# mcbuehler/DeepSEE

Measured on AMD Instinct MI355X. Metric: train-step images/sec (G+D fwd+bwd), 8x 32->256 bs=8, higher is better.
Workload: dtype fp32

## Files before the change

deepsee_amd/csrc/coarse.cpp:

```cpp
#include <hip/hip_runtime.h>
#include <stdint.h>

#include <initializer_list>
#include <vector>

#include "../../include/deepsee_hip.h"

void dsee_set_error(const char* fmt, ...);

namespace {

constexpr int kHidden = 128;
constexpr long kAmaxFloats = 64 * 32;
constexpr double kWgradF16x2MinFlop = 1e9;

#define DSEE_TRY(call)          \
  do {                          \
    const int rc__ = (call);    \
    if (rc__ != DSEE_OK) return rc__; \
  } while (0)

inline size_t up256(size_t b) { return (b + 255) / 256 * 256; }

struct Arena {
// ... 45 lines not shown
                 int C, hipStream_t stream) {
  const int has_t = nl.table != nullptr, ld = kHidden + (has_t ? 32 : 0), rows = 2 * C;
  if (!b.tab_ready) DSEE_TRY(dsee_onehot_conv3x3_pack(nl.w_shared, b.tab, kHidden, label_nc, stream));
  DSEE_TRY(dsee_onehot_conv3x3_fwd(labels, b.tab, nl.b_shared, b.cat, N, lab_h, lab_w, shift, label_nc, kHidden, ld, 0, 1,
                                   has_t ? kHidden : -1, b.amax_cat, has_t ? 1.0f : 0.0f, stream));
  if (from == kStatsOfX)
    DSEE_TRY(dsee_norm_stats(x, N, H * W, C, 1, eps, momentum, b.mean, b.invstd, nl.running_mean, nl.running_var, b.stats, stream));
  else if (from == kStatsOfParts)
    DSEE_TRY(dsee_norm_stats_finalize_parts(part, dsee_stats_part_rows((long)N * (H / 4) * (W / 4) * (C / 4)), C, eps, momentum,
                                            b.mean, b.invstd, nl.running_mean, nl.running_var, stream));
  else
    DSEE_TRY(dsee_norm_eval_stats(nl.running_mean, nl.running_var, C, eps, b.mean, b.invstd, stream));
  if (b.wp_direct) {
    const dsee_conv_geom g = {N, H, W, ld, H, W, rows, 3, 3, 1, -1, 1, 0, 0, 1};
    return dsee_conv2d_modulate_fwd(&g, b.cat, b.wp_direct, nl.table, kHidden, nl.bias_packed, x, b.mean, b.invstd, b.out_h,
                                    b.out_scale, C, nl.add_one, slope, stream);
  }
  DSEE_TRY(dsee_wino43_input_f16x2(b.cat, b.v2, N, H, W, ld, b.amax_cat, DSEE_WINO_V_BOUND, stream));
  if (!b.u_ready && !b.u_bound_ready) {
    DSEE_TRY(dsee_absmax(nl.w2a, (long)rows * kHidden * 9, b.amax_u, stream));
    if (has_t) DSEE_TRY(dsee_absmax(nl.table, (long)N * 9 * rows * 32, b.amax_u, stream));
  }
  if (has_t)
    DSEE_TRY(dsee_wino43_weights_table(nl.w2a, nl.table, reinterpret_cast<float*>(b.u2), N, rows, kHidden, 2, b.amax_u, stream));
  else if (!b.u_ready)
    DSEE_TRY(dsee_wino43_weights(nl.w2a, reinterpret_cast<float*>(b.u2), rows, kHidden, 0, 2, b.amax_u, stream));
  return dsee_spade_fused_fwd(b.v2, b.u2, b.amax_cat, DSEE_WINO_V_BOUND, b.amax_u, nl.bias_packed, x, b.mean, b.invstd, b.out_h,
                              b.out_scale, N, H, W, C, rows, ld, has_t ? N : 1, nl.add_one, slope, b.amax_h, b.amax_xhat, b.sign_mask,
                              stream);
}

int gemm_nt(const void* a2, const void* b2, float* c, long M, int Nn, int K, long rpg, int brows, const float* amax_a, float bound,
            const float* amax_b, hipStream_t st) {
  if (Nn % 256 == 0 && K % 32 == 0) return dsee_gemm_f16x2_pre_w4(a2, b2, c, M, Nn, K, rpg, brows, amax_a, bound, amax_b, st);
  return dsee_gemm_f16x2_pre(a2, b2, c, M, Nn, K, rpg, brows, amax_a, bound, amax_b, st);
}

int wino_conv3x3_product(const float* h, const float* amax_h, const float* w, float* amax_w, uint16_t* v2, uint16_t* u2, float* m,
                         bool choose_gemm, int N, int H, int W, int C, hipStream_t stream) {
  const long T = (long)N * (H / 4) * (W / 4);
  DSEE_TRY(dsee_absmax(w, (long)C * C * 9, amax_w, stream));
  DSEE_TRY(dsee_wino43_weights(w, reinterpret_cast<float*>(u2), C, C, 0, 2, amax_w, stream));
  DSEE_TRY(dsee_wino43_input_f16x2(h, v2, N, H, W, C, amax_h, DSEE_WINO_V_BOUND, stream));
  return (choose_gemm ? gemm_nt : dsee_gemm_f16x2_pre)(v2, u2, m, 36 * T, C, C, T, C, amax_h, DSEE_WINO_V_BOUND, amax_w, stream);
}

struct InferScratch {
  size_t norm_bytes;
  float *h, *dx0, *stat, *amax_h, *amax_w, *m;
  uint16_t *v2, *u2;
};
// ... 902 lines not shown
```

deepsee_amd/csrc/spade_fused.hip:

```cpp
#include <stdlib.h>

#include <type_traits>
#include <utility>

#include "dsee_common.h"

#ifndef DSEE_FUSED_ABL
#define DSEE_FUSED_ABL 0
#endif

#ifndef DSEE_FUSED_SCHED
#define DSEE_FUSED_SCHED 0
#endif

#ifndef DSEE_FUSED_SET_A
#define DSEE_FUSED_SET_A 4
#endif
#define DSEE_FUSED_SET_B (32 / DSEE_FUSED_SET_A)

#ifndef DSEE_FUSED_W16_DEFAULT
#define DSEE_FUSED_W16_DEFAULT 0
#endif

namespace {
// ... 31 lines not shown
    tg = (sup / rh) * DSEE_FUSED_SET_A + (in / DSEE_FUSED_SET_B);
    rg = (int)(sup % rh) * DSEE_FUSED_SET_B + (in % DSEE_FUSED_SET_B);
  } else {
    tg = l / rgn;
    rg = (int)(l % rgn);
  }
  const long t0 = tg * 64;
  const int n = (int)(t0 / a.tpi);
  const int g = a.G > 1 ? n : 0;

  const float sv = dsee_pow2_scale(a.v_bound * dsee_amax_read(a.amax_v));
  const float su = dsee_pow2_scale(dsee_amax_read(a.amax_u));
  const float oscale = 1.f / (sv * su);

  const int dr = 8 * wave + (lane >> 3);
  const int dcc = (lane & 7) ^ ((dr >> 1) & 7);
  const int dslab = dcc >> 2;
  const unsigned dlo = (unsigned)(dr * 64 + (dcc & 3) * 16);
  const unsigned voffu = dlo + (unsigned)dslab * (unsigned)a.u_slab_bytes;
  const unsigned voffv = dlo + (unsigned)dslab * (unsigned)a.v_slab_bytes;
  const unsigned voffu_l = dslab ? 0xFFFFFFF0u : voffu, voffv_l = dslab ? 0xFFFFFFF0u : voffv;
  const __amdgpu_buffer_rsrc_t rsu = __builtin_amdgcn_make_buffer_rsrc((void*)uniform_ptr(a.U2), 0, (int)a.u_bytes, 0x00020000);
  const __amdgpu_buffer_rsrc_t rsv = __builtin_amdgcn_make_buffer_rsrc((void*)uniform_ptr(a.V2), 0, (int)a.v_bytes, 0x00020000);
  const unsigned PU = (unsigned)(a.G * a.u_group_bytes), PV = (unsigned)(a.T * 64);
  const unsigned QU = (unsigned)(2 * a.u_slab_bytes), QV = (unsigned)(2 * a.v_slab_bytes);
  const unsigned base_u = (unsigned)((long)g * a.u_group_bytes + (long)rg * 4096), base_v = (unsigned)(t0 * 64);
  auto dma_u = [&](int par, int pc, unsigned opos) {
    unsigned char* dst = smem + (par * NP + pc) * PIECE + wave * 1024;
    __builtin_amdgcn_raw_ptr_buffer_load_lds(rsu, (__attribute__((address_space(3))) void*)dst, 16,
                                             (HALF_LAST && pc == NP - 1) ? voffu_l : voffu, opos + pc * QU, 0, 0);
  };
  auto dma_v = [&](int par, int pc, unsigned opos) {
    unsigned char* dst = smem + UREG + (par * NP + pc) * PIECE + wave * 1024;
    __builtin_amdgcn_raw_ptr_buffer_load_lds(rsv, (__attribute__((address_space(3))) void*)dst, 16,
                                             (HALF_LAST && pc == NP - 1) ? voffv_l : voffv, opos + pc * QV, 0, 0);
  };

  const int fi = lane & 15, oc = lane >> 4;
  auto foff = [&](int r, int t) {
    const int chunk = PK ? 4 * t + oc : 4 * (oc >> 1) + 2 * t + (oc & 1);
    return (unsigned)((8 * r + (chunk ^ ((r >> 1) & 7))) * 16);
  };
  const int rga = 16 * wq + fi, rtv = 16 * wt + fi;
  const unsigned au0 = foff(rga, 0), au1 = foff(rga, 1), au0h = au0 + 7 * PIECE, au1h = au1 + 7 * PIECE;
  const unsigned av0 = UREG + foff(rtv, 0), av1 = UREG + foff(rtv, 1), av0h = av0 + 7 * PIECE, av1h = av1 + 7 * PIECE;
  struct Frag {
    u32x4 g0, g1, b0, b1, v0, v1;
  };
  auto ldf = [&](Frag& f, auto par_c, auto pc_c) {
    constexpr int so = (decltype(par_c)::value * NP + decltype(pc_c)::value) * PIECE;
    constexpr bool hi = so >= 7 * PIECE;
    constexpr int io = hi ? so - 7 * PIECE : so;
    static_assert(io >= 0 && io + 4096 + PIECE <= 65536, "window");
// ... 437 lines not shown
  } else {
    tg = l / rgn;
    rg = (int)(l % rgn);
  }
  const long t0 = tg * 64;
  const int n = (int)(t0 / a.tpi);
  const int g = a.G > 1 ? n : 0;

  const float sv = dsee_pow2_scale(a.v_bound * dsee_amax_read(a.amax_v));
  const float su = dsee_pow2_scale(dsee_amax_read(a.amax_u));
  const float oscale = 1.f / (sv * su);

  const bool dma_v = wave >= 8;
  const int dw = wave & 7;
  const int dr = 8 * dw + (lane >> 3);
  const int dcc = (lane & 7) ^ ((dr >> 1) & 7);
  const int dslab = dcc >> 2;
  const unsigned dlo = (unsigned)(dr * 64 + (dcc & 3) * 16);
  const unsigned slab_bytes = (unsigned)(dma_v ? a.v_slab_bytes : a.u_slab_bytes);
  const unsigned voff = dlo + (unsigned)dslab * slab_bytes;
  const unsigned voff_l = dslab ? 0xFFFFFFF0u : voff;
  const __amdgpu_buffer_rsrc_t rs = __builtin_amdgcn_make_buffer_rsrc(
      (void*)uniform_ptr(dma_v ? a.V2 : a.U2), 0, (int)(dma_v ? a.v_bytes : a.u_bytes), 0x00020000);
  const unsigned PP_ = dma_v ? (unsigned)(a.T * 64) : (unsigned)(a.G * a.u_group_bytes);
  const unsigned QQ_ = 2 * slab_bytes;
  const unsigned base_o = dma_v ? (unsigned)(t0 * 64) : (unsigned)((long)g * a.u_group_bytes + (long)rg * 4096);
  unsigned char* const dbase = smem + (dma_v ? UREG : 0) + dw * 1024;
  auto dma = [&](int par, int pc, unsigned opos) {
    unsigned char* dst = dbase + (par * NP + pc) * PIECE;
    __builtin_amdgcn_raw_ptr_buffer_load_lds(rs, (__attribute__((address_space(3))) void*)dst, 16,
                                             (HALF_LAST && pc == NP - 1) ? voff_l : voff, opos + pc * QQ_, 0, 0);
  };

  const int fi = lane & 15, oc = lane >> 4;
  auto foff = [&](int r, int t) {
    const int chunk = PK ? 4 * t + oc : 4 * (oc >> 1) + 2 * t + (oc & 1);
    return (unsigned)((8 * r + (chunk ^ ((r >> 1) & 7))) * 16);
  };
  const int rga = 16 * wb + fi, rtv = 16 * wt + fi;
  const unsigned au0 = foff(rga, 0), au1 = foff(rga, 1);
  const unsigned av0 = UREG + foff(rtv, 0), av1 = UREG + foff(rtv, 1);
  struct Frag {
    u32x4 a0, a1, v0, v1;
  };
  auto ldf = [&](Frag& f, auto par_c, auto pc_c) {
    constexpr int so = (decltype(par_c)::value * NP + decltype(pc_c)::value) * PIECE;
    constexpr bool hi = so >= 7 * PIECE;
    constexpr int io = hi ? so - 7 * PIECE : so;
    static_assert(io >= 0 && io + PIECE <= 65536, "window");
    const unsigned w0 = hi ? 7 * PIECE : 0;
    f.a0 = *reinterpret_cast<const u32x4*>(smem + (au0 + w0) + io);
    f.a1 = *reinterpret_cast<const u32x4*>(smem + (au1 + w0) + io);
    f.v0 = *reinterpret_cast<const u32x4*>(smem + (av0 + w0) + io);
    f.v1 = *reinterpret_cast<const u32x4*>(smem + (av1 + w0) + io);
// ... 237 lines not shown
    }
  }
  if (a.amax_xhat) {
#pragma unroll
    for (int o = 32; o > 0; o >>= 1) xmax = fmaxf(xmax, __shfl_xor(xmax, o, 64));
    if (lane == 0) {
      unsigned* line = reinterpret_cast<unsigned*>(a.amax_xhat + ((blockIdx.x * 16 + wave) & (DSEE_AMAX_LINES - 1)) * DSEE_AMAX_STRIDE);
      const unsigned bits = __builtin_bit_cast(unsigned, xmax);
      if (bits > __hip_atomic_load(line, __ATOMIC_RELAXED, __HIP_MEMORY_SCOPE_AGENT)) atomicMax(line, bits);
    }
  }
#endif
}

}

static float* g_fused_stamps = nullptr;

#if DSEE_FUSED_ABL
extern "C" void dsee_fused_set_stamps(float* p) { g_fused_stamps = p; }
#endif


static int spade_fused_launch(bool packed, const void* V2, const void* U2, const float* amax_cat, float v_bound,
                              const float* amax_u, const float* bias_packed, const float* x, const float* mean,
                              const float* invstd, float* out_h, float* out_scale, int N, int H, int W, int C, int rows, int K,
                              int groups, int stat_groups, float add_one, float slope, float* amax_h, float* amax_xhat,
                              unsigned* sign_mask, hipStream_t st) {
  DSEE_CHECK_ARG(V2 && U2 && amax_cat && amax_u && x && mean && invstd && out_h);
  DSEE_CHECK_ARG(rows == 2 * C && C % 32 == 0 && H % 4 == 0 && W % 4 == 0 && (K == 128 || K == 160));
  DSEE_CHECK_ARG(groups == 1 || groups == N);
  DSEE_CHECK_ARG(stat_groups == 1 || stat_groups == N);
  const int tpi = (H / 4) * (W / 4);
  DSEE_CHECK_ARG(tpi % 64 == 0);
  const long T = (long)N * tpi;
  FusedArgs a;
  a.V2 = (const unsigned char*)V2;
  a.U2 = (const unsigned char*)U2;
  a.amax_v = amax_cat;
  a.amax_u = amax_u;
  a.bias = bias_packed;
  a.x = x;
  a.mean = mean;
  a.invstd = invstd;
  a.stat_ld = stat_groups == 1 ? 0 : C;
  a.out = out_h;
  a.scale = out_scale;
  a.mask = sign_mask;
  a.cshift = 0;
  while ((4 << a.cshift) < 4 * C) ++a.cshift;
  a.cshift += 2;
  DSEE_CHECK_ARG(!sign_mask || (C & (C - 1)) == 0);
  DSEE_CHECK_ARG((long)N * H * W * C < (1L << 30));
  a.amax_h = amax_h;
  a.amax_xhat = amax_xhat;
  a.T = T;
  a.v_slab_bytes = 36L * T * 64;
  a.u_slab_bytes = (long)rows * 64;
  const int kslab = packed ? 32 : 16;
  a.u_group_bytes = (long)(K / kslab) * rows * 64;
  const long vb = a.v_slab_bytes * (K / kslab), ub = a.u_group_bytes * 36 * groups;
  DSEE_CHECK_ARG(vb < 0xFFFFFFF0L && ub < 0xFFFFFFF0L);
  a.v_bytes = (unsigned)vb;
  a.u_bytes = (unsigned)ub;
  a.tpi = tpi;
  a.tw = W / 4;
  a.H = H;
  a.W = W;
  a.C = C;
  a.rows = rows;
  a.G = groups;
  a.v_bound = v_bound;
  a.add_one = add_one;
  a.slope = slope;
  a.stamps = g_fused_stamps;
  const long ntile = (T / 64) * (rows / 64);
  DSEE_CHECK_ARG(ntile < 0x7FFFFFFF);
  const int np = packed ? (K + 63) / 64 : K / 32;
  const int rd = packed ? 3 : 2;
  const size_t lds = (size_t)rd * np * 16384;
  const char* const w16_env = getenv("DSEE_FUSED_W16");
  const int w16 = w16_env ? atoi(w16_env) : DSEE_FUSED_W16_DEFAULT;
#define DSEE_FUSED_K(KERNEL, THREADS, NP, WS, PKD)                                                                   \
  do {                                                                                                               \
    static bool attr_done = false;                                                                                   \
    if (!attr_done) {                                                                                                \
      hipError_t e = hipFuncSetAttribute(reinterpret_cast<const void*>(&KERNEL<NP, WS, PKD, (PKD ? 3 : 2)>),         \
                                         hipFuncAttributeMaxDynamicSharedMemorySize, (int)lds);                     \
      if (e != hipSuccess) {                                                                                         \
        dsee_set_error("hipFuncSetAttribute(%zu bytes of LDS): %s", lds, hipGetErrorString(e));                     \
        return DSEE_ELAUNCH;                                                                                         \
      }                                                                                                              \
      attr_done = true;                                                                                              \
    }                                                                                                                \
    KERNEL<NP, WS, PKD, (PKD ? 3 : 2)><<<(int)ntile, THREADS, lds, st>>>(a);                                         \
  } while (0)
#define DSEE_FUSED(NP, WS, PKD)                                                                                      \
  do {                                                                                                               \
    if (w16)                                                                                                         \
      DSEE_FUSED_K(spade_fused_fwd16_kernel, 1024, NP, WS, PKD);                                                     \
    else                                                                                                             \
// ... 2 lines not shown
  if (packed) {
    if (np == 3) {
      if (out_scale) DSEE_FUSED(3, true, true); else DSEE_FUSED(3, false, true);
    } else {
      if (out_scale) DSEE_FUSED(2, true, true); else DSEE_FUSED(2, false, true);
    }
  } else if (np == 5) {
    if (out_scale) DSEE_FUSED(5, true, false); else DSEE_FUSED(5, false, false);
  } else {
    if (out_scale) DSEE_FUSED(4, true, false); else DSEE_FUSED(4, false, false);
  }
#undef DSEE_FUSED
#undef DSEE_FUSED_K
  DSEE_LAUNCH_CHECK();
  return DSEE_OK;
}

extern "C" {

int dsee_spade_fused_fwd(const void* V2, const void* U2, const float* amax_cat, float v_bound, const float* amax_u,
                         const float* bias_packed, const float* x, const float* mean, const float* invstd, float* out_h,
                         float* out_scale, int N, int H, int W, int C, int rows, int K, int groups, float add_one,
                         float slope, float* amax_h, float* amax_xhat, uint32_t* sign_mask, hipStream_t st) {
  return spade_fused_launch(false, V2, U2, amax_cat, v_bound, amax_u, bias_packed, x, mean, invstd, out_h, out_scale, N, H, W,
                            C, rows, K, groups, 1, add_one, slope, amax_h, amax_xhat, sign_mask, st);
}

int dsee_spade_fused_fwd_f16p(const void* V1, const void* U1, const float* amax_cat, float v_bound, const float* amax_u,
                              const float* bias_packed, const float* x, const float* mean, const float* invstd, float* out_h,
                              float* out_scale, int N, int H, int W, int C, int rows, int K, int groups, float add_one,
                              float slope, float* amax_h, float* amax_xhat, uint32_t* sign_mask, hipStream_t st) {
  return spade_fused_launch(true, V1, U1, amax_cat, v_bound, amax_u, bias_packed, x, mean, invstd, out_h, out_scale, N, H, W,
                            C, rows, K, groups, 1, add_one, slope, amax_h, amax_xhat, sign_mask, st);
}

int dsee_spade_fused_fwd_sg(const void* V2, const void* U2, const float* amax_cat, float v_bound, const float* amax_u,
                            const float* bias_packed, const float* x, const float* mean, const float* invstd, float* out_h,
                            float* out_scale, int N, int H, int W, int C, int rows, int K, int groups, int stat_groups,
                            float add_one, float slope, float* amax_h, float* amax_xhat, uint32_t* sign_mask, hipStream_t st) {
  return spade_fused_launch(false, V2, U2, amax_cat, v_bound, amax_u, bias_packed, x, mean, invstd, out_h, out_scale, N, H, W,
                            C, rows, K, groups, stat_groups, add_one, slope, amax_h, amax_xhat, sign_mask, st);
}

int dsee_spade_fused_fwd_f16p_sg(const void* V1, const void* U1, const float* amax_cat, float v_bound, const float* amax_u,
                                 const float* bias_packed, const float* x, const float* mean, const float* invstd,
                                 float* out_h, float* out_scale, int N, int H, int W, int C, int rows, int K, int groups,
                                 int stat_groups, float add_one, float slope, float* amax_h, float* amax_xhat,
                                 uint32_t* sign_mask, hipStream_t st) {
  return spade_fused_launch(true, V1, U1, amax_cat, v_bound, amax_u, bias_packed, x, mean, invstd, out_h, out_scale, N, H, W,
                            C, rows, K, groups, stat_groups, add_one, slope, amax_h, amax_xhat, sign_mask, st);
}

}
```

deepsee_amd/csrc/spade_fused_args.h:

```cpp
#pragma once
#include <type_traits>
#include <utility>

#include "dsee_common.h"

namespace {

typedef _Float16 f16x8 __attribute__((ext_vector_type(8)));
typedef unsigned u32x4 __attribute__((ext_vector_type(4)));

struct FusedArgs {
  const unsigned char* V2;
  const unsigned char* U2;
  const float* amax_v;
  const float* amax_u;
  const float* bias;
  const float* x;
  const float* mean;
  const float* invstd;
  int stat_ld;
  float* out;
  float* amax_h;
  float* amax_xhat;
  float* scale;
  int cshift;
  unsigned* mask;
  long T;
  long v_slab_bytes, u_slab_bytes, u_group_bytes;
  unsigned v_bytes, u_bytes;
  int tpi, tw;
  int H, W, C, rows;
  int G;
  float v_bound, add_one, slope;
  float* stamps;
};

template <int I>
using ic = std::integral_constant<int, I>;
template <class F, int... Is>
__device__ __forceinline__ void static_for_impl(F&& f, std::integer_sequence<int, Is...>) {
  (f(ic<Is>{}), ...);
}
template <int N, class F>
__device__ __forceinline__ void static_for(F&& f) {
  static_for_impl(f, std::make_integer_sequence<int, N>{});
}

__device__ __forceinline__ const unsigned char* uniform_ptr(const unsigned char* p) {
  const unsigned long long v = (unsigned long long)p;
  const unsigned lo = __builtin_amdgcn_readfirstlane((unsigned)v), hi = __builtin_amdgcn_readfirstlane((unsigned)(v >> 32));
  return (const unsigned char*)(((unsigned long long)hi << 32) | lo);
// ... 5 lines not shown
```

deepsee_amd/csrc/winograd.hip:

```cpp
#include "dsee_common.h"
#include "dsee_rng.h"

namespace {

typedef unsigned short u16x4 __attribute__((ext_vector_type(4)));
__device__ __forceinline__ void split3(float x, unsigned short (&h)[3]) {
  const __bf16 b0 = (__bf16)x;
  const float r1 = x - (float)b0;
  const __bf16 b1 = (__bf16)r1;
  const __bf16 b2 = (__bf16)(r1 - (float)b1);
  h[0] = __builtin_bit_cast(unsigned short, b0);
  h[1] = __builtin_bit_cast(unsigned short, b1);
  h[2] = __builtin_bit_cast(unsigned short, b2);
}
__device__ __forceinline__ size_t split_index(size_t row, int k, size_t rows, int p) {
  return (((size_t)(k >> 4) * rows + row) * 3 + p) * 16 + (k & 15);
}
__device__ __forceinline__ void store_split4(unsigned short* base, size_t row, int k, size_t rows, const f32x4& v) {
  unsigned short h[4][3];
#pragma unroll
  for (int e = 0; e < 4; ++e) split3(v[e], h[e]);
#pragma unroll
  for (int p = 0; p < 3; ++p) {
    const u16x4 w = {h[0][p], h[1][p], h[2][p], h[3][p]};
// ... 1015 lines not shown
#pragma unroll
  for (int j = 0; j < 8; ++j) {
    const float x = v[j] * sc;
    h0[j] = (_Float16)x;
    h1[j] = (_Float16)(x - (float)h0[j]);
  }
  auto pk = [](_Float16 a, _Float16 b) {
    return (unsigned)__builtin_bit_cast(unsigned short, a) | ((unsigned)__builtin_bit_cast(unsigned short, b) << 16);
  };
  const dsee_u32x4 w0 = {pk(h0[0], h0[1]), pk(h0[2], h0[3]), pk(h0[4], h0[5]), pk(h0[6], h0[7])};
  _Float16* Uh = reinterpret_cast<_Float16*>(U);
  if (split == 2) {
    const dsee_u32x4 w1 = {pk(h1[0], h1[1]), pk(h1[2], h1[3]), pk(h1[4], h1[5]), pk(h1[6], h1[7])};
    _Float16* o = Uh + block * per * 2 + (((size_t)(k0 >> 4) * rows + row) * 2) * 16 + (k0 & 15);
    *reinterpret_cast<dsee_u32x4*>(o) = w0;
    *reinterpret_cast<dsee_u32x4*>(o + 16) = w1;
  } else if (split == 3) {
    *reinterpret_cast<dsee_u32x4*>(Uh + block * per + ((size_t)(k0 >> 4) * rows + row) * 16 + (k0 & 15)) = w0;
  } else {
    *reinterpret_cast<dsee_u32x4*>(Uh + block * per + ((size_t)(k0 >> 5) * rows + row) * 32 + (k0 & 31)) = w0;
  }
}

__global__ __launch_bounds__(256) void wino43_weight_table8_kernel(const float* __restrict__ w2a, const float* __restrict__ table,
                                                                   float* __restrict__ U, int N, int rows, int ca, int Kpad,
                                                                   int split, const float* __restrict__ amax) {
  const unsigned K8 = (unsigned)Kpad >> 3;
  const size_t per = (size_t)rows * Kpad;
  const long total = (long)N * rows * K8;
  const float sc = split >= 2 ? dsee_pow2_scale(dsee_amax_read(amax)) : 1.f;
  for (long i = blockIdx.x * (long)blockDim.x + threadIdx.x; i < total; i += (long)gridDim.x * blockDim.x) {
    const unsigned iu = (unsigned)i, rr = iu / K8, n = rr / (unsigned)rows;
    const int k0 = (int)(iu - rr * K8) * 8, row = (int)(rr - n * (unsigned)rows);
    float g[8][9];
    if (k0 < ca) {
      const f32x4* src = reinterpret_cast<const f32x4*>(w2a + ((size_t)row * ca + k0) * 9);
#pragma unroll
      for (int q = 0; q < 18; ++q) {
        const f32x4 v = src[q];
#pragma unroll
        for (int e = 0; e < 4; ++e) g[(q * 4 + e) / 9][(q * 4 + e) % 9] = v[e];
      }
    } else if (k0 < ca + 32) {
#pragma unroll
      for (int tap = 0; tap < 9; ++tap) {
        const float* src = table + (((size_t)n * 9 + tap) * rows + row) * 32 + (k0 - ca);
        const f32x4 a = *reinterpret_cast<const f32x4*>(src), b = *reinterpret_cast<const f32x4*>(src + 4);
#pragma unroll
        for (int e = 0; e < 4; ++e) {
          g[e][tap] = a[e];
          g[4 + e][tap] = b[e];
        }
      }
    } else {
#pragma unroll
      for (int j = 0; j < 8; ++j)
#pragma unroll
        for (int tap = 0; tap < 9; ++tap) g[j][tap] = 0.f;
    }
    ggt8(g, [&](int xi, const float (&v)[8]) { store_u8(U, split, (size_t)xi * N + n, per, rows, Kpad, row, k0, sc, v); });
  }
}

__global__ __launch_bounds__(256) void wino43_weight8_kernel(const float* __restrict__ w, float* __restrict__ U, int Cout, int Cin,
                                                             int rows, int Kpad, int transpose_flip, int split,
                                                             const float* __restrict__ amax, long w_stride, long u_stride) {
  w += (size_t)blockIdx.y * w_stride;
  U += (size_t)blockIdx.y * u_stride;
  if (amax) amax += (size_t)blockIdx.y * (DSEE_AMAX_LINES * DSEE_AMAX_STRIDE);
  const unsigned K8 = (unsigned)Kpad >> 3;
  const size_t per = (size_t)rows * Kpad;
  const long total = (long)rows * K8;
  const float sc = split >= 2 ? dsee_pow2_scale(dsee_amax_read(amax)) : 1.f;
  const int R = transpose_flip ? Cin : Cout, K = transpose_flip ? Cout : Cin;
  for (long i = blockIdx.x * (long)blockDim.x + threadIdx.x; i < total; i += (long)gridDim.x * blockDim.x) {
    const unsigned iu = (unsigned)i, row = iu / K8;
    const int k0 = (int)(iu - row * K8) * 8;
    float g[8][9];
#pragma unroll
    for (int j = 0; j < 8; ++j) {
      const int k = k0 + j;
      const bool ok = (int)row < R && k < K;
      const int co = transpose_flip ? k : (int)row, ci = transpose_flip ? (int)row : k;
// ... 401 lines not shown
                                   int stat_groups, float add_one, float slope, const float* mscale, hipStream_t st) {
  DSEE_CHECK_ARG(stat_groups == 1 || stat_groups == N);
  const int stat_ld = stat_groups == 1 ? 0 : C;
  DSEE_CHECK_ARG(wino_items32(N, H, W, C));
  DSEE_CHECK_ARG(M && x && mean && invstd && out_h && C % 64 == 0 && rows == 2 * C);
  DSEE_CHECK_ARG(H % 4 == 0 && W % 4 == 0);
  DSEE_CHECK_ARG((long)N * (H / 4) * (W / 4) * rows * 4 < 0xFFFFFFF0L);
  const int grid = wgrid((long)N * (H / 4) * (W / 4) * (C / 4));
  if (mscale)
    wino43_output_modulate_kernel<<<grid, 256, 0, st>>>(reinterpret_cast<const _Float16*>(M), bias_packed, x, mean, invstd,
                                                        out_h, out_scale, N, H, W, C, rows, add_one, slope, mscale, stat_ld);
  else
    wino43_output_modulate_kernel<<<grid, 256, 0, st>>>(M, bias_packed, x, mean, invstd, out_h, out_scale, N, H, W, C, rows,
                                                        add_one, slope, nullptr, stat_ld);
  DSEE_LAUNCH_CHECK();
  return DSEE_OK;
}

int dsee_wino43_weights_table(const float* w2a, const float* table, float* U, int N, int rows, int ca, int split,
                              const float* amax_w, hipStream_t st) {
  DSEE_CHECK_ARG(table && U && (ca == 0 || w2a) && ca % 32 == 0 && rows % 128 == 0 && (split < 2 || amax_w));
  const int Kpad = dsee_conv_kpad(1, 1, ca + 32);
  if (split != 1 && Kpad % 8 == 0)
    wino43_weight_table8_kernel<<<wgrid((long)N * rows * Kpad / 8), 256, 0, st>>>(w2a, table, U, N, rows, ca, Kpad, split,
                                                                                  amax_w);
  else
    wino43_weight_table_kernel<<<wgrid((long)N * rows * Kpad), 256, 0, st>>>(w2a, table, U, N, rows, ca, Kpad, split,
                                                                             amax_w);
  DSEE_LAUNCH_CHECK();
  return DSEE_OK;
}

}
```

deepsee_amd/ops.py:

```python
import os
import ctypes as C

import threading
from collections import namedtuple
from typing import NamedTuple, Optional

import torch

from . import lib as L
from .plan import KernelPlan, DEFAULT_PLAN, current as P

LRELU_SLOPE = 0.2
BN_EPS = 1e-5
BN_MOMENTUM = 0.1
SN_EPS = 1e-12
NHIDDEN = 128

_scratch = {}

PROFILE = None
PROFILE_BYTES = {}
PROFILE_OPERAND_GB = 0.0


# ... 1705 lines not shown
def _norm_cat(w_sh, b_sh, labels, shift, n, h, w, has_a, has_t, cat_ups):
    nc, ca = labels.nc, (NHIDDEN if has_a else 0)
    ld = ca + (32 if has_t else 0)
    cat, actv_low = new(n, h, w, ld), None
    cat_amax = amax_slot()
    if has_a:
        tab = new(9, nc, NHIDDEN)
        L.call("onehot_conv3x3_pack", w_sh.contiguous(), tab, NHIDDEN, nc)
        if cat_ups:
            assert not has_t and ld == NHIDDEN
            actv_low = new(n, h >> cat_ups, w >> cat_ups, NHIDDEN)
            L.call("onehot_conv3x3_fwd", labels.t, tab, b_sh, actv_low, n, labels.h, labels.w, shift, nc, NHIDDEN,
                   NHIDDEN, 0, 1, -1, cat_amax, 0.0)
            L.call("upsample_noise_fwd", actv_low, None, None, cat, n, h, w, NHIDDEN, cat_ups)
        else:
            L.call("onehot_conv3x3_fwd", labels.t, tab, b_sh, cat, n, labels.h, labels.w, shift, nc, NHIDDEN, ld, 0,
                   1, ca if has_t else -1, cat_amax, 1.0 if has_t else 0.0)
    elif has_t:
        L.call("label_onehot", labels.t, cat, n, labels.h, labels.w, shift, ld, ca)
        cat_amax = None
    return cat, cat_amax, actv_low


def _norm_u(w2a, table, nb, rows, ca, kp, split):
    if table is None:
        return _wino_u(w2a, rows, ca, False, rows, kp, split)
    ua = weight_amax(w2a, table) if split >= 2 else None
    u = _i16(36 * nb * rows * kp * {1: 3, 2: 2, 3: 1, 4: 1}[split]) if split else new(36, nb, rows, kp)
    L.call("wino43_weights_table", w2a, table, u, nb, rows, ca, int(split), ua)
    return u, ua


def _norm_keeps_v(scale, nb, n, ld, rows):
    return P().keep_v and scale is not None and nb == n and _wgrad_mode(ld, rows) == 2


def _norm_product_fused(cat, cat_amax, w2a, table, ca, b2, x, mean, invstd, out, scale, add_one, rows, nb):
    (n, h, w, c), ld, sg = x.shape, cat.shape[3], stat_groups(mean)
    kp, t = L.kpad(1, 1, ld), n * (h // 4) * (w // 4)
    ac = cat_amax if cat_amax is not None else tensor_amax(cat)
    pk = P().half
    v2 = WinoOperand(_i16(36 * t * ld * (1 if pk else 2)), ac, F16P if pk else F16X2)
    L.call("wino43_input_f16p" if pk else "wino43_input_f16x2", cat, v2.data, n, h, w, ld, ac, FUSED_V_BOUND)
    u, ua = _norm_u(w2a, table, n, rows, ca, kp, 4 if pk else 2)
    if PROFILE is not None:
        global PROFILE_OPERAND_GB
        PROFILE_OPERAND_GB += (t // 64) * (rows // 64) * 36 * 2 * 64 * ld * 4.0 / 1e9
    with _timed("spade_fused_fwd", 2.0 * 36 * t * ld * rows,
                4.0 * 36 * t * ld + 4.0 * n * h * w * c * (3 if scale is not None else 2)):
        hm = amax_slot()
        xm = amax_slot() if scale is not None else None
        smask = (torch.empty(n * h * w * (c // 32), dtype=torch.int32, device=x.device)
                 if (scale is not None and P().sign_mask and (c & (c - 1)) == 0) else None)
        _call_sg("spade_fused_fwd_f16p" if pk else ("spade_fused_fwd_w4" if (P().fused_w4 and sg == 1) else
                                                    "spade_fused_fwd"), sg,
                 (v2.data, u, ac, FUSED_V_BOUND, ua, b2.contiguous(), x, mean, invstd, out, scale, n,
                  h, w, c, rows, ld, n if table is not None else 1), (float(add_one), LRELU_SLOPE, hm, xm, smask))
        tag_amax(out, hm)
    keep = v2 if _norm_keeps_v(scale, nb, n, ld, rows) else None
    if keep is not None and not P().presplit_a:
        keep = WinoOperand(new(36, t, ld), amax_slot(), FP32)
        L.call("wino43_input", cat, keep.data, n, h, w, ld, keep.amax)
    return keep, xm, smask, ac


def _norm_product_wino(cat, w2a, table, ca, b2, x, mean, invstd, out, scale, add_one, rows, nb):
    (n, h, w, c), ld, sg = x.shape, cat.shape[3], stat_groups(mean)
    kp, b2c, split = L.kpad(1, 1, ld), b2.contiguous(), _split_kind(ld, rows)
    keep = [] if _norm_keeps_v(scale, nb, n, ld, rows) else None
    for n0 in range(0, n, nb):
        u, ua = _norm_u(w2a, None if table is None else table[n0:n0 + nb], nb, rows, ca, kp, split)
        m, ms = _wino_vgemm(cat[n0:n0 + nb], nb, h, w, ld, u, rows, rows, kp, table is not None, split, keep, ua)
        px = nb * h * w
        with _timed("spade_modulate_fused", 0.0,
                    (2.0 if split == 3 else 4.0) * 36 * (px // 16) * rows + 4.0 * px * c * (3 if scale is not None else 2)):
            mc, ic = (mean, invstd) if sg == 1 else (mean[n0:n0 + nb], invstd[n0:n0 + nb])
            _call_sg("wino43_output_modulate", 1 if sg == 1 else nb,
                     (m, b2c, x[n0:n0 + nb], mc, ic, out[n0:n0 + nb], scale[n0:n0 + nb] if scale is not None else None, nb, h,
                      w, c, rows), (float(add_one), LRELU_SLOPE, ms))
    return keep[0] if keep else None
# ... 283 lines not shown
```

deepsee_amd/plan.py:

```python
import contextlib
import dataclasses
import threading
from typing import Any, Optional


@dataclasses.dataclass(frozen=True)
class KernelPlan:
    winograd: bool = True
    winograd_wgrad: bool = True
    winograd_mod: bool = True
    gemm_split: bool = True
    gemm_af32: bool = True
    keep_v: bool = True
    gemm_f16x2: bool = True
    half: bool = False
    half_norms: bool = True
    presplit_a: bool = True
    gemm_w4: bool = True
    dgrad_s2_parity: bool = True
    presplit_min_tiles: int = 512
    conv_halo_f16: bool = True
    onehot_wgrad_mfma: bool = True
    conv_amax_out: bool = True
    presplit_dm: bool = True
    presplit_gb: bool = True
    dout_sums: bool = True
    adjoint_dgrad: bool = True
    fuse_noise: bool = True
    thin_gemm: bool = True
    share_stats: bool = True
    producer_stats: bool = True
    fuse_dm: bool = True
    fused_norm: bool = True
    fused_w4: bool = False
    sign_mask: bool = True
    defer_act: bool = True
    branch_streams: bool = False
    conv_f16x2_min_flop: float = 1e9
    sync_bn: Optional[Any] = None

    def replace(self, **changes):
        return dataclasses.replace(self, **changes)

    @contextlib.contextmanager
    def active(self):
        prev = getattr(_tls, "plan", None)
        _tls.plan = self
        try:
            yield self
        finally:
            _tls.plan = prev

    @classmethod
    def fields(cls):
        return [f.name for f in dataclasses.fields(cls)]


# ... 35 lines not shown
```

include/deepsee_hip.h:

```cpp
#ifndef DEEPSEE_HIP_H
#define DEEPSEE_HIP_H

#include <stddef.h>
#include <stdint.h>

#ifdef __cplusplus
extern "C" {
#endif

#ifndef __HIP_INCLUDE_HIP_HIP_RUNTIME_API_H__
typedef struct ihipStream_t* hipStream_t;
#endif

#define DSEE_OK 0
#define DSEE_EINVAL (-1)
#define DSEE_ELAUNCH (-2)
#define DSEE_EUNSUPPORTED (-3)

#define DSEE_ACT_NONE 0
#define DSEE_ACT_LRELU 1
#define DSEE_ACT_RELU 2
#define DSEE_ACT_TANH 3
#define DSEE_ACT_MASK 4

// ... 113 lines not shown
int dsee_bilinear_up_u8(const uint8_t* src, long src_image_stride, long src_row_stride, int S, uint8_t* dst, int N, int H,
                        int W, long dst_image_stride, long dst_row_stride, int dst_x_offset, hipStream_t stream);
int dsee_style_explore(const float* s0, const float* s1, const int32_t* src0, const int32_t* src1, const float* alpha,
                       const float* beta, const float* gamma, const float* noise, const uint8_t* mask, float* out, int B, int n,
                       int nc, int S, int clamp, int recurrent, hipStream_t stream);
int dsee_nhwc_to_nchw_tiled(const float* x, float* y, int B, int n, int H, int W, int cs, int merge, int pair0, int pairs,
                            hipStream_t stream);
int dsee_selftest_lds_poison(float* sink, hipStream_t stream);
int dsee_conv2d_fwd_grouped(const dsee_conv_geom* g, const float* in, const float* w_packed, long group_stride,
                            float* out, hipStream_t stream);
int dsee_wino43_output_modulate(const float* M, const float* bias_packed, const float* x, const float* mean,
                                const float* invstd, float* out_h, float* out_scale, int N, int H, int W, int C,
                                int rows, float add_one, float slope, const float* mscale, hipStream_t stream);
int dsee_wino43_weights_table(const float* w2a, const float* table, float* U, int N, int rows, int ca, int split,
                              const float* amax_w, hipStream_t stream);
#define DSEE_WINO_V_BOUND 100.0f
int dsee_wino43_input_f16x2(const float* x, void* V2, int N, int H, int W, int C, const float* amax_x, float bound,
                            hipStream_t stream);
int dsee_spade_fused_fwd(const void* V2, const void* U2, const float* amax_cat, float v_bound, const float* amax_u,
                         const float* bias_packed, const float* x, const float* mean, const float* invstd, float* out_h,
                         float* out_scale, int N, int H, int W, int C, int rows, int K, int groups, float add_one,
                         float slope, float* amax_h, float* amax_xhat, uint32_t* sign_mask,
                         hipStream_t stream);
size_t dsee_wino43_wgrad_table_workspace(long T, int N, int ca, int rows);
int dsee_wino43_wgrad_table(const float* V, const float* dM, float* workspace, size_t workspace_bytes, float* dw2a,
                            float* dtable, long T, int N, int ca, int rows, int L, int split, const float* amax_v,
                            const float* amax_dm, hipStream_t stream);
int dsee_wino43_dout(const float* dy, float* dM, int N, int H, int W, int C, float* amax, hipStream_t stream);
#define DSEE_WINO_DM_BOUND 1.0f
size_t dsee_wino43_dout_f16x2_workspace(void);
int dsee_wino43_dout_f16x2(const float* dy, void* dM2, int N, int H, int W, int C, const float* amax_dy, float bound,
                           float* workspace, float* dbias, float* dnoise0, uint64_t seed0, uint64_t offset0,
                           float* dnoise1, uint64_t seed1, uint64_t offset1, hipStream_t stream);
size_t dsee_wino43_dout_sums_workspace(int C);
int dsee_wino43_dout_sums(const float* dy, float* dM, int N, int H, int W, int C, float* amax, float* workspace,
                          float* dbias, float* dnoise0, uint64_t seed0, uint64_t offset0, float* dnoise1, uint64_t seed1,
                          uint64_t offset1, hipStream_t stream);
int dsee_wino43_input_adjoint(const float* dV, const float* mask, int mask_ld, float* dx, int N, int H, int W, int C,
                              const float* dvscale, float* amax_dx, hipStream_t stream);
size_t dsee_wino43_wgrad_workspace(long T, int Cin_stored, int Cout_stored);
int dsee_wino43_wgrad(const float* V, const float* dM, float* workspace, size_t workspace_bytes, float* dw_oihw,
                      long T, int Cin_stored, int Cout_stored, int Cout, int Cin, int split, const float* amax_v,
                      const float* amax_dm, hipStream_t stream);
int dsee_wino43_input_split_t(const float* x, void* V3t, int N, int H, int W, int C, hipStream_t stream);
int dsee_wino43_dout_split_t(const float* dy, void* dM3t, int N, int H, int W, int C, hipStream_t stream);
int dsee_gemm_bf16x3_tn_f32(const float* P, const float* Q, float* C, int groups, long T, int rows_p, int rows_q, int ldc,
// ... 396 lines not shown
```

Baseline: 93.13.

## Share the w2a Winograd weight block across images in fused SPADE forward

The transformed weight operand U for the table-conditioned SPADE conv used to be built per image, duplicating the shared w2a part N times. A new shared layout stores the w2a K-slabs once per Winograd position and keeps only the per-image table slab (the last 32 K) separately. The fused kernel's DMA offsets now send the last K piece to the per-image table slab. This cuts weight-transform work, U memory and L2/HBM traffic, at the cost of extra offset arithmetic and a new code path gated by plan.shared_u.

```diff
diff --git a/deepsee_amd/csrc/coarse.cpp b/deepsee_amd/csrc/coarse.cpp
--- a/deepsee_amd/csrc/coarse.cpp
+++ b/deepsee_amd/csrc/coarse.cpp
@@ -91,11 +91,12 @@
     if (has_t) DSEE_TRY(dsee_absmax(nl.table, (long)N * 9 * rows * 32, b.amax_u, stream));
   }
   if (has_t)
-    DSEE_TRY(dsee_wino43_weights_table(nl.w2a, nl.table, reinterpret_cast<float*>(b.u2), N, rows, kHidden, 2, b.amax_u, stream));
+    DSEE_TRY(dsee_wino43_weights_table_shared(nl.w2a, nl.table, reinterpret_cast<float*>(b.u2), N, rows, kHidden, 2, b.amax_u,
+                                              stream));
   else if (!b.u_ready)
     DSEE_TRY(dsee_wino43_weights(nl.w2a, reinterpret_cast<float*>(b.u2), rows, kHidden, 0, 2, b.amax_u, stream));
   return dsee_spade_fused_fwd(b.v2, b.u2, b.amax_cat, DSEE_WINO_V_BOUND, b.amax_u, nl.bias_packed, x, b.mean, b.invstd, b.out_h,
-                              b.out_scale, N, H, W, C, rows, ld, has_t ? N : 1, nl.add_one, slope, b.amax_h, b.amax_xhat, b.sign_mask,
+                              b.out_scale, N, H, W, C, rows, ld, has_t ? -N : 1, nl.add_one, slope, b.amax_h, b.amax_xhat, b.sign_mask,
                               stream);
 }
 
diff --git a/deepsee_amd/csrc/spade_fused.hip b/deepsee_amd/csrc/spade_fused.hip
--- a/deepsee_amd/csrc/spade_fused.hip
+++ b/deepsee_amd/csrc/spade_fused.hip
@@ -77,13 +77,15 @@
   const unsigned voffu_l = dslab ? 0xFFFFFFF0u : voffu, voffv_l = dslab ? 0xFFFFFFF0u : voffv;
   const __amdgpu_buffer_rsrc_t rsu = __builtin_amdgcn_make_buffer_rsrc((void*)uniform_ptr(a.U2), 0, (int)a.u_bytes, 0x00020000);
   const __amdgpu_buffer_rsrc_t rsv = __builtin_amdgcn_make_buffer_rsrc((void*)uniform_ptr(a.V2), 0, (int)a.v_bytes, 0x00020000);
-  const unsigned PU = (unsigned)(a.G * a.u_group_bytes), PV = (unsigned)(a.T * 64);
+  const unsigned PU = (unsigned)a.u_pos_bytes, PV = (unsigned)(a.T * 64);
   const unsigned QU = (unsigned)(2 * a.u_slab_bytes), QV = (unsigned)(2 * a.v_slab_bytes);
-  const unsigned base_u = (unsigned)((long)g * a.u_group_bytes + (long)rg * 4096), base_v = (unsigned)(t0 * 64);
+  const unsigned QUL = (unsigned)(a.u_last_off + (long)g * a.u_last_img);
+  const unsigned base_u = (unsigned)((long)g * a.u_img_bytes + (long)rg * 4096), base_v = (unsigned)(t0 * 64);
   auto dma_u = [&](int par, int pc, unsigned opos) {
     unsigned char* dst = smem + (par * NP + pc) * PIECE + wave * 1024;
     __builtin_amdgcn_raw_ptr_buffer_load_lds(rsu, (__attribute__((address_space(3))) void*)dst, 16,
-                                             (HALF_LAST && pc == NP - 1) ? voffu_l : voffu, opos + pc * QU, 0, 0);
+                                             (HALF_LAST && pc == NP - 1) ? voffu_l : voffu,
+                                             opos + (pc == NP - 1 ? QUL : pc * QU), 0, 0);
   };
   auto dma_v = [&](int par, int pc, unsigned opos) {
     unsigned char* dst = smem + UREG + (par * NP + pc) * PIECE + wave * 1024;
@@ -567,14 +569,16 @@
   const unsigned voff_l = dslab ? 0xFFFFFFF0u : voff;
   const __amdgpu_buffer_rsrc_t rs = __builtin_amdgcn_make_buffer_rsrc(
       (void*)uniform_ptr(dma_v ? a.V2 : a.U2), 0, (int)(dma_v ? a.v_bytes : a.u_bytes), 0x00020000);
-  const unsigned PP_ = dma_v ? (unsigned)(a.T * 64) : (unsigned)(a.G * a.u_group_bytes);
+  const unsigned PP_ = dma_v ? (unsigned)(a.T * 64) : (unsigned)a.u_pos_bytes;
   const unsigned QQ_ = 2 * slab_bytes;
-  const unsigned base_o = dma_v ? (unsigned)(t0 * 64) : (unsigned)((long)g * a.u_group_bytes + (long)rg * 4096);
+  const unsigned QQL_ = dma_v ? (NP - 1) * QQ_ : (unsigned)(a.u_last_off + (long)g * a.u_last_img);
+  const unsigned base_o = dma_v ? (unsigned)(t0 * 64) : (unsigned)((long)g * a.u_img_bytes + (long)rg * 4096);
   unsigned char* const dbase = smem + (dma_v ? UREG : 0) + dw * 1024;
   auto dma = [&](int par, int pc, unsigned opos) {
     unsigned char* dst = dbase + (par * NP + pc) * PIECE;
     __builtin_amdgcn_raw_ptr_buffer_load_lds(rs, (__attribute__((address_space(3))) void*)dst, 16,
-                                             (HALF_LAST && pc == NP - 1) ? voff_l : voff, opos + pc * QQ_, 0, 0);
+                                             (HALF_LAST && pc == NP - 1) ? voff_l : voff,
+                                             opos + (pc == NP - 1 ? QQL_ : pc * QQ_), 0, 0);
   };
 
   const int fi = lane & 15, oc = lane >> 4;
@@ -858,7 +862,7 @@
 #endif
 
 
-static int spade_fused_launch(bool packed, const void* V2, const void* U2, const float* amax_cat, float v_bound,
+static int spade_fused_launch(bool packed, bool shared_u, const void* V2, const void* U2, const float* amax_cat, float v_bound,
                               const float* amax_u, const float* bias_packed, const float* x, const float* mean,
                               const float* invstd, float* out_h, float* out_scale, int N, int H, int W, int C, int rows, int K,
                               int groups, int stat_groups, float add_one, float slope, float* amax_h, float* amax_xhat,
@@ -867,6 +871,7 @@
   DSEE_CHECK_ARG(rows == 2 * C && C % 32 == 0 && H % 4 == 0 && W % 4 == 0 && (K == 128 || K == 160));
   DSEE_CHECK_ARG(groups == 1 || groups == N);
   DSEE_CHECK_ARG(stat_groups == 1 || stat_groups == N);
+  DSEE_CHECK_ARG(!shared_u || (!packed && groups == N && (K - 32) % 32 == 0));
   const int tpi = (H / 4) * (W / 4);
   DSEE_CHECK_ARG(tpi % 64 == 0);
   const long T = (long)N * tpi;
@@ -895,7 +900,19 @@
   a.u_slab_bytes = (long)rows * 64;
   const int kslab = packed ? 32 : 16;
   a.u_group_bytes = (long)(K / kslab) * rows * 64;
-  const long vb = a.v_slab_bytes * (K / kslab), ub = a.u_group_bytes * 36 * groups;
+  const int np = packed ? (K + 63) / 64 : K / 32;
+  if (shared_u) {
+    a.u_pos_bytes = (long)((K - 32) / 16 + 2 * groups) * a.u_slab_bytes;
+    a.u_img_bytes = 0;
+    a.u_last_off = (long)((K - 32) / 16) * a.u_slab_bytes;
+    a.u_last_img = 2 * a.u_slab_bytes;
+  } else {
+    a.u_pos_bytes = (long)groups * a.u_group_bytes;
+    a.u_img_bytes = a.u_group_bytes;
+    a.u_last_off = (long)(np - 1) * 2 * a.u_slab_bytes;
+    a.u_last_img = 0;
+  }
+  const long vb = a.v_slab_bytes * (K / kslab), ub = a.u_pos_bytes * 36;
   DSEE_CHECK_ARG(vb < 0xFFFFFFF0L && ub < 0xFFFFFFF0L);
   a.v_bytes = (unsigned)vb;
   a.u_bytes = (unsigned)ub;
@@ -912,7 +929,6 @@
   a.stamps = g_fused_stamps;
   const long ntile = (T / 64) * (rows / 64);
   DSEE_CHECK_ARG(ntile < 0x7FFFFFFF);
-  const int np = packed ? (K + 63) / 64 : K / 32;
   const int rd = packed ? 3 : 2;
   const size_t lds = (size_t)rd * np * 16384;
   const char* const w16_env = getenv("DSEE_FUSED_W16");
@@ -961,15 +977,16 @@
                          const float* bias_packed, const float* x, const float* mean, const float* invstd, float* out_h,
                          float* out_scale, int N, int H, int W, int C, int rows, int K, int groups, float add_one,
                          float slope, float* amax_h, float* amax_xhat, uint32_t* sign_mask, hipStream_t st) {
-  return spade_fused_launch(false, V2, U2, amax_cat, v_bound, amax_u, bias_packed, x, mean, invstd, out_h, out_scale, N, H, W,
-                            C, rows, K, groups, 1, add_one, slope, amax_h, amax_xhat, sign_mask, st);
+  const bool su = groups < 0;
+  return spade_fused_launch(false, su, V2, U2, amax_cat, v_bound, amax_u, bias_packed, x, mean, invstd, out_h, out_scale, N, H, W,
+                            C, rows, K, su ? -groups : groups, 1, add_one, slope, amax_h, amax_xhat, sign_mask, st);
 }
 
 int dsee_spade_fused_fwd_f16p(const void* V1, const void* U1, const float* amax_cat, float v_bound, const float* amax_u,
                               const float* bias_packed, const float* x, const float* mean, const float* invstd, float* out_h,
                               float* out_scale, int N, int H, int W, int C, int rows, int K, int groups, float add_one,
                               float slope, float* amax_h, float* amax_xhat, uint32_t* sign_mask, hipStream_t st) {
-  return spade_fused_launch(true, V1, U1, amax_cat, v_bound, amax_u, bias_packed, x, mean, invstd, out_h, out_scale, N, H, W,
+  return spade_fused_launch(true, false, V1, U1, amax_cat, v_bound, amax_u, bias_packed, x, mean, invstd, out_h, out_scale, N, H, W,
                             C, rows, K, groups, 1, add_one, slope, amax_h, amax_xhat, sign_mask, st);
 }
 
@@ -977,7 +994,7 @@
                             const float* bias_packed, const float* x, const float* mean, const float* invstd, float* out_h,
                             float* out_scale, int N, int H, int W, int C, int rows, int K, int groups, int stat_groups,
                             float add_one, float slope, float* amax_h, float* amax_xhat, uint32_t* sign_mask, hipStream_t st) {
-  return spade_fused_launch(false, V2, U2, amax_cat, v_bound, amax_u, bias_packed, x, mean, invstd, out_h, out_scale, N, H, W,
+  return spade_fused_launch(false, false, V2, U2, amax_cat, v_bound, amax_u, bias_packed, x, mean, invstd, out_h, out_scale, N, H, W,
                             C, rows, K, groups, stat_groups, add_one, slope, amax_h, amax_xhat, sign_mask, st);
 }
 
@@ -986,7 +1003,7 @@
                                  float* out_h, float* out_scale, int N, int H, int W, int C, int rows, int K, int groups,
                                  int stat_groups, float add_one, float slope, float* amax_h, float* amax_xhat,
                                  uint32_t* sign_mask, hipStream_t st) {
-  return spade_fused_launch(true, V1, U1, amax_cat, v_bound, amax_u, bias_packed, x, mean, invstd, out_h, out_scale, N, H, W,
+  return spade_fused_launch(true, false, V1, U1, amax_cat, v_bound, amax_u, bias_packed, x, mean, invstd, out_h, out_scale, N, H, W,
                             C, rows, K, groups, stat_groups, add_one, slope, amax_h, amax_xhat, sign_mask, st);
 }
 
diff --git a/deepsee_amd/csrc/spade_fused_args.h b/deepsee_amd/csrc/spade_fused_args.h
--- a/deepsee_amd/csrc/spade_fused_args.h
+++ b/deepsee_amd/csrc/spade_fused_args.h
@@ -27,6 +27,7 @@
   unsigned* mask;
   long T;
   long v_slab_bytes, u_slab_bytes, u_group_bytes;
+  long u_pos_bytes, u_img_bytes, u_last_off, u_last_img;
   unsigned v_bytes, u_bytes;
   int tpi, tw;
   int H, W, C, rows;
diff --git a/deepsee_amd/csrc/winograd.hip b/deepsee_amd/csrc/winograd.hip
--- a/deepsee_amd/csrc/winograd.hip
+++ b/deepsee_amd/csrc/winograd.hip
@@ -1061,16 +1061,19 @@
   }
 }
 
+template <bool SHARED>
 __global__ __launch_bounds__(256) void wino43_weight_table8_kernel(const float* __restrict__ w2a, const float* __restrict__ table,
                                                                    float* __restrict__ U, int N, int rows, int ca, int Kpad,
                                                                    int split, const float* __restrict__ amax) {
   const unsigned K8 = (unsigned)Kpad >> 3;
   const size_t per = (size_t)rows * Kpad;
-  const long total = (long)N * rows * K8;
+  const long total = (long)(SHARED ? 1 : N) * rows * K8;
   const float sc = split >= 2 ? dsee_pow2_scale(dsee_amax_read(amax)) : 1.f;
   for (long i = blockIdx.x * (long)blockDim.x + threadIdx.x; i < total; i += (long)gridDim.x * blockDim.x) {
-    const unsigned iu = (unsigned)i, rr = iu / K8, n = rr / (unsigned)rows;
-    const int k0 = (int)(iu - rr * K8) * 8, row = (int)(rr - n * (unsigned)rows);
+    const unsigned iu = (unsigned)i, rr = iu / K8;
+    const int ks = (int)(iu - rr * K8) * 8;
+    const unsigned n = SHARED ? (ks < ca ? 0u : (unsigned)(ks - ca) >> 5) : rr / (unsigned)rows;
+    const int k0 = SHARED ? (ks < ca ? ks : ca + ((ks - ca) & 31)) : ks, row = (int)(rr - (SHARED ? 0u : n * (unsigned)rows));
     float g[8][9];
     if (k0 < ca) {
       const f32x4* src = reinterpret_cast<const f32x4*>(w2a + ((size_t)row * ca + k0) * 9);
@@ -1097,7 +1100,9 @@
 #pragma unroll
         for (int tap = 0; tap < 9; ++tap) g[j][tap] = 0.f;
     }
-    ggt8(g, [&](int xi, const float (&v)[8]) { store_u8(U, split, (size_t)xi * N + n, per, rows, Kpad, row, k0, sc, v); });
+    ggt8(g, [&](int xi, const float (&v)[8]) {
+      store_u8(U, split, SHARED ? (size_t)xi : (size_t)xi * N + n, per, rows, Kpad, row, ks, sc, v);
+    });
   }
 }
 
@@ -1545,8 +1550,8 @@
   DSEE_CHECK_ARG(table && U && (ca == 0 || w2a) && ca % 32 == 0 && rows % 128 == 0 && (split < 2 || amax_w));
   const int Kpad = dsee_conv_kpad(1, 1, ca + 32);
   if (split != 1 && Kpad % 8 == 0)
-    wino43_weight_table8_kernel<<<wgrid((long)N * rows * Kpad / 8), 256, 0, st>>>(w2a, table, U, N, rows, ca, Kpad, split,
-                                                                                  amax_w);
+    wino43_weight_table8_kernel<false><<<wgrid((long)N * rows * Kpad / 8), 256, 0, st>>>(w2a, table, U, N, rows, ca, Kpad,
+                                                                                         split, amax_w);
   else
     wino43_weight_table_kernel<<<wgrid((long)N * rows * Kpad), 256, 0, st>>>(w2a, table, U, N, rows, ca, Kpad, split,
                                                                              amax_w);
@@ -1554,4 +1559,18 @@
   return DSEE_OK;
 }
 
-}
+int dsee_wino43_weights_table_shared(const float* w2a, const float* table, float* U, int N, int rows, int ca, int split,
+                                     const float* amax_w, hipStream_t st) {
+  DSEE_CHECK_ARG(table && U && w2a && amax_w && N >= 1 && ca >= 32 && ca % 32 == 0 && rows >= 64 && rows % 64 == 0);
+  if (split != 2) {
+    dsee_set_error("dsee_wino43_weights_table_shared: split = %d (the shared layout exists for the two-term fp16 form only)", split);
+    return DSEE_EUNSUPPORTED;
+  }
+  const long Kv = ca + 32L * N;
+  DSEE_CHECK_ARG(rows * Kv / 8 < (1L << 31));
+  wino43_weight_table8_kernel<true><<<wgrid(rows * Kv / 8), 256, 0, st>>>(w2a, table, U, N, rows, ca, (int)Kv, 2, amax_w);
+  DSEE_LAUNCH_CHECK();
+  return DSEE_OK;
+}
+
+}
diff --git a/deepsee_amd/ops.py b/deepsee_amd/ops.py
--- a/deepsee_amd/ops.py
+++ b/deepsee_amd/ops.py
@@ -1751,10 +1751,15 @@
     return cat, cat_amax, actv_low
 
 
-def _norm_u(w2a, table, nb, rows, ca, kp, split):
+def _norm_u(w2a, table, nb, rows, ca, kp, split, shared=False):
     if table is None:
         return _wino_u(w2a, rows, ca, False, rows, kp, split)
     ua = weight_amax(w2a, table) if split >= 2 else None
+    if shared:
+        assert split == 2 and kp == ca + 32
+        u = _i16(36 * (ca // 16 + 2 * nb) * rows * 32)
+        L.call("wino43_weights_table_shared", w2a, table, u, nb, rows, ca, 2, ua)
+        return u, ua
     u = _i16(36 * nb * rows * kp * {1: 3, 2: 2, 3: 1, 4: 1}[split]) if split else new(36, nb, rows, kp)
     L.call("wino43_weights_table", w2a, table, u, nb, rows, ca, int(split), ua)
     return u, ua
@@ -1771,7 +1776,8 @@
     pk = P().half
     v2 = WinoOperand(_i16(36 * t * ld * (1 if pk else 2)), ac, F16P if pk else F16X2)
     L.call("wino43_input_f16p" if pk else "wino43_input_f16x2", cat, v2.data, n, h, w, ld, ac, FUSED_V_BOUND)
-    u, ua = _norm_u(w2a, table, n, rows, ca, kp, 4 if pk else 2)
+    su = (P().shared_u and table is not None and not pk and not P().fused_w4 and sg == 1 and ca >= 32 and ca % 32 == 0)
+    u, ua = _norm_u(w2a, table, n, rows, ca, kp, 4 if pk else 2, su)
     if PROFILE is not None:
         global PROFILE_OPERAND_GB
         PROFILE_OPERAND_GB += (t // 64) * (rows // 64) * 36 * 2 * 64 * ld * 4.0 / 1e9
@@ -1784,7 +1790,8 @@
         _call_sg("spade_fused_fwd_f16p" if pk else ("spade_fused_fwd_w4" if (P().fused_w4 and sg == 1) else
                                                     "spade_fused_fwd"), sg,
                  (v2.data, u, ac, FUSED_V_BOUND, ua, b2.contiguous(), x, mean, invstd, out, scale, n,
-                  h, w, c, rows, ld, n if table is not None else 1), (float(add_one), LRELU_SLOPE, hm, xm, smask))
+                  h, w, c, rows, ld, (-n if su else n) if table is not None else 1),
+                 (float(add_one), LRELU_SLOPE, hm, xm, smask))
         tag_amax(out, hm)
     keep = v2 if _norm_keeps_v(scale, nb, n, ld, rows) else None
     if keep is not None and not P().presplit_a:
diff --git a/deepsee_amd/plan.py b/deepsee_amd/plan.py
--- a/deepsee_amd/plan.py
+++ b/deepsee_amd/plan.py
@@ -33,6 +33,7 @@
     fuse_dm: bool = True
     fused_norm: bool = True
     fused_w4: bool = False
+    shared_u: bool = True
     sign_mask: bool = True
     defer_act: bool = True
     branch_streams: bool = False
diff --git a/include/deepsee_hip.h b/include/deepsee_hip.h
--- a/include/deepsee_hip.h
+++ b/include/deepsee_hip.h
@@ -159,6 +159,8 @@
                          float* out_scale, int N, int H, int W, int C, int rows, int K, int groups, float add_one,
                          float slope, float* amax_h, float* amax_xhat, uint32_t* sign_mask,
                          hipStream_t stream);
+int dsee_wino43_weights_table_shared(const float* w2a, const float* table, float* U, int N, int rows, int ca, int split,
+                                     const float* amax_w, hipStream_t stream);
 size_t dsee_wino43_wgrad_table_workspace(long T, int N, int ca, int rows);
 int dsee_wino43_wgrad_table(const float* V, const float* dM, float* workspace, size_t workspace_bytes, float* dw2a,
                             float* dtable, long T, int N, int ca, int rows, int L, int split, const float* amax_v,
```

Measured after the change: 94.31 (median of 6 runs). 1.01x the previous value.
